# dwu4/fhe-si

Measured on AMD Instinct MI355X. Metric: homomorphic ciphertext-mults/sec (incl. relinearize) at n=2^14, logQ=512, higher is better.
Workload: dtype u32 (every transformed row is a row of 4-byte residues modulo a prime below 2^30: tensor half over primes of 30 bits, key switch over four of 30; coefficients are u64 limbs)

## Files before the change

fhe-si_amd/csrc/capi_ctx.hip:

```cpp
#include "capi_common.h"

int ws_reserve(fhesi_ctx* ctx, int slot, size_t bytes, void** out) {
  if (ctx->ws_bytes[slot] < bytes) {
    if (ctx->ws[slot]) { HIP_TRY(hipStreamSynchronize(ctx->stream)); HIP_TRY(hipFree(ctx->ws[slot])); ctx->ws[slot] = nullptr; ctx->ws_bytes[slot] = 0; }
    size_t want = bytes + (bytes >> 3) + 4096;
    if (hipMalloc(&ctx->ws[slot], want) != hipSuccess) {
      (void)hipGetLastError();
      ctx->ws[slot] = nullptr;
      if (hipMalloc(&ctx->ws[slot], bytes) != hipSuccess) {
        (void)hipGetLastError();
        ctx->ws[slot] = nullptr;
        ctx->ws_oom = true;
        FHESI_FAIL("workspace slot %d: hipMalloc of %zu bytes failed", slot, bytes);
      }
      want = bytes;
    }
    ctx->ws_bytes[slot] = want;
  }
  *out = ctx->ws[slot];
  if (ctx->ws_poison && bytes) HIP_TRY(hipMemsetAsync(ctx->ws[slot], 0xA5, bytes, ctx->stream));
  return 0;
}

int upload_idx(fhesi_ctx* ctx, const std::vector<int>& idx, int** d_out) {
// ... 34 lines not shown
  twt.assign(n, Shoup2{0, 0});
  for (int i = 0; i < 32; ++i) twt[i] = tw[i];
  for (int u = 0; u < 5; ++u)
    for (int x = 0; x < (1 << u); ++x)
      for (int p1 = 0; p1 < 32; ++p1) twt[32 + ((1 << u) - 1 + x) * 32 + p1] = tw[(1 << (5 + u)) + (p1 << u) + x];
  for (int u = 0; u < R; ++u)
    for (int x = 0; x < (1 << u); ++x)
      for (int jl = 0; jl < 1024; ++jl) twt[1024 + (i64)((1 << u) - 1 + x) * 1024 + jl] = tw[(1 << (10 + u)) + ((i64)hm::brv(jl, 10) << u) + x];
}
static void to_q63(std::vector<Shoup2>& t, u64 q) {
  for (auto& e : t) e.wp = hm::shoup63(e.w, q);
}

thread_local bool g_fhesi_internal_ctx = false;

struct OptDesc { const char* name; const char* env; size_t off; bool wide; };
static const OptDesc kOptions[] = {
  {"ks_direct", "FHESI_KS_DIRECT", offsetof(CtxOptions, ks_direct), false},
  {"ks_residues", "FHESI_KS_RESIDUES", offsetof(CtxOptions, ks_residues), false},
  {"ks_aux60", "FHESI_KS_AUX60", offsetof(CtxOptions, ks_aux60), false},
  {"crt_exact", "FHESI_CRT_EXACT", offsetof(CtxOptions, crt_exact), false},
  {"crt_skip_cleanup", "FHESI_CRT_SKIP_CLEANUP", offsetof(CtxOptions, crt_skip_cleanup), false},
  {"lanes", "FHESI_LANES", offsetof(CtxOptions, lanes), false},
  {"stagger", "FHESI_STAGGER", offsetof(CtxOptions, stagger), false},
  {"batch_chunk", "FHESI_BATCH_CHUNK", offsetof(CtxOptions, batch_chunk), true},
  {"wave_operands", "FHESI_WAVE_OPERANDS", offsetof(CtxOptions, wave_operands), true},
  {"stage_chunk_bytes", "FHESI_STAGE_CHUNK_BYTES", offsetof(CtxOptions, stage_chunk_bytes), true},
  {"wave_single", "FHESI_WAVE_SINGLE", offsetof(CtxOptions, wave_single), false},
  {"tensor32", "FHESI_TENSOR32", offsetof(CtxOptions, tensor32), false},
  {"tensor_bits", "FHESI_TENSOR_BITS", offsetof(CtxOptions, tensor_bits), false},
  {"crt32_mfma", "FHESI_CRT32_MFMA", offsetof(CtxOptions, crt32_mfma), false},
  {"dot32_k4", "FHESI_DOT32_K4", offsetof(CtxOptions, dot32_k4), false},
  {"parts_words", "FHESI_PARTS_WORDS", offsetof(CtxOptions, parts_words), false},
  {"hoist_dot", "FHESI_HOIST_DOT", offsetof(CtxOptions, hoist_dot), false},
  {"automorph_rows", "FHESI_AUTOMORPH_ROWS", offsetof(CtxOptions, automorph_rows), false},
  {"ks_long_keys", "FHESI_KS_LONG_KEYS", offsetof(CtxOptions, ks_long_keys), false},
  {"host_chunk", "FHESI_HOST_CHUNK", offsetof(CtxOptions, host_chunk), true},
  {"host_threads", "FHESI_HOST_THREADS", offsetof(CtxOptions, host_threads), false},
};
static void opt_store(CtxOptions* o, const OptDesc& d, long long v) {
  if (d.wide) *(long long*)((char*)o + d.off) = v; else *(int*)((char*)o + d.off) = (int)v;
}
static long long opt_load(const CtxOptions* o, const OptDesc& d) {
  return d.wide ? *(const long long*)((const char*)o + d.off) : (long long)*(const int*)((const char*)o + d.off);
}
extern "C" int fhesi_ctx_set_option(fhesi_ctx* c, const char* name, int64_t value) {
  if (!c || !name) FHESI_FAIL("set_option: null argument");
  for (const OptDesc& d : kOptions)
    if (!strcmp(d.name, name)) { opt_store(&c->opt, d, value); return 0; }
  FHESI_FAIL("set_option: unknown option '%s'", name);
}
extern "C" int fhesi_ctx_get_option(const fhesi_ctx* c, const char* name, int64_t* value) {
  if (!c || !name || !value) FHESI_FAIL("get_option: null argument");
  for (const OptDesc& d : kOptions)
    if (!strcmp(d.name, name)) { *value = opt_load(&c->opt, d); return 0; }
  FHESI_FAIL("get_option: unknown option '%s'", name);
}
extern "C" int fhesi_ctx_copy_options(fhesi_ctx* dst, const fhesi_ctx* src) {
  if (!dst || !src) FHESI_FAIL("copy_options: null argument");
  dst->opt = src->opt;
  return 0;
}

extern "C" int fhesi_ctx_create(fhesi_ctx** out, int64_t m, int32_t nprimes, const uint64_t* q, const uint64_t* root, int32_t device) {
  if (!out) FHESI_FAIL("null output pointer");
  *out = nullptr;
// ... 317 lines not shown
```

fhe-si_amd/csrc/fhesi_internal.h:

```cpp
#pragma once
#include <hip/hip_runtime.h>
#include <cstdint>
#include <cmath>
#include <cstdio>
#include <map>
#include <string>
#include <atomic>
#include <vector>
#include <algorithm>
#include <type_traits>
#include "hostbig.h"
#include "ct_wide.h"

typedef unsigned int u32;

void fhesi_set_error(const char* fmt, ...);
#define FHESI_FAIL(...) do { fhesi_set_error(__VA_ARGS__); return 1; } while (0)
#define HIP_TRY(expr) do { hipError_t e__ = (expr); if (e__ != hipSuccess) { fhesi_set_error("%s failed: %s (%s:%d)", #expr, hipGetErrorString(e__), __FILE__, __LINE__); return 1; } } while (0)
#define FHESI_OP_SET_ 4
#define FHESI_WS_SLOTS 16
#define FHESI_TRY(expr) do { int r__ = (expr); if (r__) return r__; } while (0)

template <int C, int... Rest, class F> static inline void with_limb_class(int n, F&& f) {
  if constexpr (sizeof...(Rest) == 0) f(std::integral_constant<int, C>{});
// ... 45 lines not shown
  std::vector<u64> P, halfP;
};

struct BluesteinTables;
struct fhesi_aux32;

enum { PROF_NTT_FWD = 0, PROF_NTT_INV = 1, PROF_RNS = 2, PROF_TENSOR = 3, PROF_CRT = 4, PROF_DIGITS = 5, PROF_DOT = 6, PROF_EW = 7, PROF_NTT_FWD_DIGITS_MAIN = 8, PROF_NCLASS = 9,
       PROF_PLAIN_SUM = 15  };
enum { PROF_NAME_CRT_EXACT = PROF_NCLASS, PROF_NAME_KS_RECOMBINE, PROF_NAME_RNS_GENERIC, PROF_NAME_MODSWITCH, PROF_NAME_DIGITS, PROF_NNAME };
struct ProfRec { int cls; double units; hipEvent_t e0, e1; };

struct CtxOptions {
  long long host_chunk = 0;
  int host_threads = 0;
  int ks_long_keys = 0;
  int ks_direct = 0;
  int ks_residues = 0;
  int ks_aux60 = 0;
  int crt_exact = 0;
  int crt_skip_cleanup = 0;
  int lanes = 1;
  int stagger = 0;
  long long batch_chunk = 0;
  long long wave_operands = 0;
  long long stage_chunk_bytes = 0;
  int wave_single = 1;
  int automorph_rows = 0;
  int tensor32 = 1;
  int tensor_bits = 30;
  int crt32_mfma = 1;
  int dot32_k4 = 1;
  int hoist_dot = 0;
  int parts_words = 1;
};

struct fhesi_ctx {
  CtxOptions opt;
  int live_handles = 0;
  int device = 0;
  hipStream_t stream = nullptr;
  hipEvent_t ev0 = nullptr, ev1 = nullptr;
  i64 m = 0, phim = 0;
  int L = 0;
  bool pow2 = false;
  int n_big_primes = 0;
  bool has_small_prime = false;
  int logn = 0;
  i64 lin_q = 0;
  bool lin_prime = false;
  i64 lin_s = 0;
  bool phi_two_term = false;
  int lin_lg = 0;
  std::vector<u64> q, root;
  std::vector<int> zms_idx;
  std::vector<i64> phi;
  std::vector<PrimeConst> pc;
  PrimeConst* d_pc = nullptr;
  Shoup2* d_tw_fwd = nullptr;
  Shoup2* d_tw_inv = nullptr;
  Shoup2* d_twt_fwd = nullptr;
  Shoup2* d_twt_inv = nullptr;
  Shoup2* d_twt_fwd_sub = nullptr;
  Shoup2* d_head_tw = nullptr;
  Shoup2* d_tail_fwd = nullptr;
  Shoup2* d_sub_fold = nullptr;
  int* d_zms_idx = nullptr;
// ... 346 lines not shown
```

fhe-si_amd/csrc/kernels_aux32.hip:

```cpp
#include "fhesi_internal.h"

#include "ntt32_core.inc"

__global__ void __launch_bounds__(256) ntt32_head_kernel(u32* __restrict__ rows, i64 count, int nslots, int a0, Aux32Primes pr, Aux32Head hd) {
  const i64 row = blockIdx.y;
  const int a = a0 + (int)(row % nslots);
  const u32 p = pr.p[a];
  u32* g = rows + row * 2 * A32_N;
  for (i64 e = (i64)blockIdx.x * blockDim.x + threadIdx.x; e < A32_N; e += (i64)gridDim.x * blockDim.x) {
    u32 x = g[e];
    const u32 t = mul_lazy32(g[e + A32_N], hd.head[a], p);
    x = x >= 2 * p ? x - 2 * p : x;
    g[e] = x + t;
    g[e + A32_N] = x + 2 * p - t;
  }
}
__global__ void __launch_bounds__(256) ntt32_tail_kernel(u32* __restrict__ rows, i64 count, int nslots, int a0, Aux32Primes pr, Aux32Head hd) {
  const i64 row = blockIdx.y;
  const int a = a0 + (int)(row % nslots);
  const u32 p = pr.p[a];
  u32* g = rows + row * 2 * A32_N;
  for (i64 e = (i64)blockIdx.x * blockDim.x + threadIdx.x; e < A32_N; e += (i64)gridDim.x * blockDim.x) {
    const u32 A = g[e], B = g[e + A32_N];
    u32 s0 = mul_lazy32(A + B, hd.tail_sum[a], p), s1 = mul_lazy32(A + p - B, hd.tail_dif[a], p);
// ... 59 lines not shown
void aux32_free(fhesi_ctx* ctx) {
  if (!ctx->aux32) return;
  ctx->aux32->tab.release();
  delete ctx->aux32;
  ctx->aux32 = nullptr;
}

int launch_ntt32_fwd(fhesi_ctx* ctx, u32* d_rows, i64 count, int nslots, int a0) {
  FHESI_TRY(aux32_init(ctx));
  if (!count) return 0;
  const fhesi_aux32* x = ctx->aux32;
  const int S = x->S;
  if (S >= 2) { if (!launch_ntt32_head_pass(ctx->stream, S, d_rows, count * nslots, nslots, a0, x->tab)) FHESI_FAIL("ntt32: no kernel for rows of 2^%d", A32_LOGN + S); }
  else if (S) ntt32_head_kernel<<<dim3(16, (unsigned)(count * nslots)), 256, 0, ctx->stream>>>(d_rows, count, nslots, a0, x->pr, x->hd);
  if (S) HIP_TRY(hipGetLastError());
  if (count > 0x7fffffff || (nslots << S) > 65535) FHESI_FAIL("ntt32: too many rows per launch");
  const dim3 grid((unsigned)count, (unsigned)(nslots << S));
  if (!a32_with_S<0, 6>(S, [&](auto s) {
    constexpr int SS = decltype(s)::value;
    PROF_KERNEL(ctx, PROF_NTT_FWD, ntt32_fwd_kernel3<false, SS>);
    ntt32_fwd_kernel3<false, SS><<<grid, A32_T, 0, ctx->stream>>>(d_rows, count, nslots, a0, x->pr, x->tab.d_fwd, Dig32Src{}, x->hd);
  })) FHESI_FAIL("ntt32: no kernel for rows of 2^%d", A32_LOGN + S);
  HIP_TRY(hipGetLastError());
  return 0;
}
int launch_ntt32_inv(fhesi_ctx* ctx, u32* d_rows, i64 count, int nslots, int a0, bool mont, bool tail) {
  FHESI_TRY(aux32_init(ctx));
  if (!count) return 0;
  const fhesi_aux32* x = ctx->aux32;
  const int S = x->S;
  ProfScope prof(ctx, PROF_NTT_INV, (double)(count * nslots));
  if (count > 0x7fffffff || (nslots << S) > 65535) FHESI_FAIL("ntt32: too many rows per launch");
  const dim3 grid((unsigned)count, (unsigned)(nslots << S));
  if (mont && S < 3) { PROF_KERNEL(ctx, PROF_NTT_INV, ntt32_inv_kernel3<true>); ntt32_inv_kernel3<true><<<grid, A32_T, 0, ctx->stream>>>(d_rows, count, nslots, a0, x->pr, x->tab.d_inv, S, nullptr); }
  else { PROF_KERNEL(ctx, PROF_NTT_INV, ntt32_inv_kernel3<false>); ntt32_inv_kernel3<false><<<grid, A32_T, 0, ctx->stream>>>(d_rows, count, nslots, a0, x->pr, x->tab.d_inv, S, nullptr); }
  HIP_TRY(hipGetLastError());
  if (S >= 2 && !tail) FHESI_FAIL("ntt32: rows of 2^16 and longer have no consumer that takes their tail stages");
  if (S && tail) {
    if (S >= 2) { if (!launch_ntt32_tail_pass(ctx->stream, S, d_rows, count * nslots, nslots, a0, x->tab, mont ? 1 : 0)) FHESI_FAIL("ntt32: no kernel for rows of 2^%d", A32_LOGN + S); }
    else ntt32_tail_kernel<<<dim3(16, (unsigned)(count * nslots)), 256, 0, ctx->stream>>>(d_rows, count, nslots, a0, x->pr, x->hd);
    HIP_TRY(hipGetLastError());
  }
  return 0;
}
int aux32_tail_consts(fhesi_ctx* ctx, uint32_t (*tw)[2], uint32_t (*twp)[2]) {
  FHESI_TRY(aux32_init(ctx));
  const fhesi_aux32* x = ctx->aux32;
  for (int a = 0; a < 4; ++a) { tw[a][0] = x->hd.tail_sum[a].w; twp[a][0] = x->hd.tail_sum[a].wp; tw[a][1] = x->hd.tail_dif[a].w; twp[a][1] = x->hd.tail_dif[a].wp; }
  return 0;
}
int launch_ntt32_fwd_digits(fhesi_ctx* ctx, const u64* d_parts, int nl, int digit_bits, int nd, i64 npolys, u32* d_out, i64 sub_units, bool wm) {
  FHESI_TRY(aux32_init(ctx));
  if (!npolys) return 0;
  const fhesi_aux32* x = ctx->aux32;
  const int S = x->S;
  ProfScope prof(ctx, PROF_NTT_FWD, (double)(npolys * nd * 4));
  ProfScope main_prof(ctx, PROF_NTT_FWD_DIGITS_MAIN, (double)(npolys * nd * 4));
  const i64 units = npolys * nd;
  if (units > 0x7fffffff) FHESI_FAIL("ntt32: too many digit rows per launch");
  if (digit_bits > 30) FHESI_FAIL("ntt32: digits of %d bits (the first stage of a digit row assumes values below 2p)", digit_bits);
  Dig32Src src{d_parts, nl, digit_bits, nd, (u32)ctx->phim, (u32)sub_units, div32_inv((u32)nd), div32_inv((u32)sub_units)};
  if (S >= 3) {
    if (!ctx->lin_q) FHESI_FAIL("ntt32: digit rows of 2^%d exist for the padded linear-convolution rings only", A32_LOGN + S);
    if (units > 65535) FHESI_FAIL("ntt32: %lld digit rows of 2^%d in one launch (at least 2 MB each: the caller's chunks are smaller)", (long long)units, A32_LOGN + S);
    void* tmp;
    FHESI_TRY(ws_reserve(ctx, 11, (size_t)units * 4 * ((size_t)A32_N << S) * 4, &tmp));
// ... 658 lines not shown
```

fhe-si_amd/csrc/kernels_tensor32.hip:

```cpp
#include "fhesi_internal.h"
#include "lin_fold.h"
#include "ntt32_core.inc"
#include "crt32_bytes.h"
#include <cmath>

struct T32Config {
  u64 lift = 0;
  int nl = 0, logQ = 0, NP = 0, R = 28, WT = 0;
  bool generic = false;
  T32Primes pr;
  u32* d_rns = nullptr;
  Tw32* d_cinv = nullptr;
  u32* d_inv57 = nullptr;
  u32* d_Mw = nullptr;
  u32* d_bytes = nullptr;
  ~T32Config() { hipFree(d_rns); hipFree(d_cinv); hipFree(d_inv57); hipFree(d_Mw); hipFree(d_bytes); }
};
struct fhesi_tensor32 {
  int S = 0;
  int bits = 30;
  hm::Ring32Consts k;
  Ring32Dev tab;
  std::vector<T32Config*> cfgs;
  T32Config* cur = nullptr;
// ... 664 lines not shown
    default: break;
  }
#undef T32_RNS
  FHESI_FAIL("tensor32: %d limbs", c->nl);
}
template <class F>
static inline void t32_with_bits(const fhesi_tensor32* x, F&& f) {
  if (x->bits == 29) f(std::integral_constant<int, 29>{}); else f(std::integral_constant<int, 30>{});
}
static int t32_fwd(fhesi_ctx* ctx, const T32Config* c, u32* d_r, i64 npolys) {
  const fhesi_tensor32* x = ctx->tensor32;
  ProfScope prof(ctx, PROF_NTT_FWD, (double)(npolys * c->NP));
  if (npolys > 0x7fffffff) FHESI_FAIL("tensor32: too many rows per launch");
  const dim3 grid((unsigned)npolys, (unsigned)(c->NP << x->S));
  if (x->S >= 3) {
    if (!launch_ntt32_head_pass(ctx->stream, x->S, d_r, npolys * c->NP, c->NP, 0, x->tab)) FHESI_FAIL("tensor32: no kernel for rows of 2^%d", A32_LOGN + x->S);
    HIP_TRY(hipGetLastError());
  }
  if (!a32_with_S<0, 6>(x->S, [&](auto s) {
    constexpr int SS = decltype(s)::value;
    t32_with_bits(x, [&](auto pb) {
      constexpr int PB = decltype(pb)::value;
      PROF_KERNEL(ctx, PROF_NTT_FWD, (ntt32_fwd_kernel3<false, SS, false, T32Primes, true, false, PB>));
      ntt32_fwd_kernel3<false, SS, false, T32Primes, true, false, PB><<<grid, A32_T, 0, ctx->stream>>>(d_r, npolys, c->NP, 0, c->pr, x->tab.d_fwd, Dig32Src{}, Aux32Head{});
    });
  })) FHESI_FAIL("tensor32: no kernel for rows of 2^%d", A32_LOGN + x->S);
  HIP_TRY(hipGetLastError());
  return 0;
}
template <bool TENSOR>
static int t32_inv(fhesi_ctx* ctx, const T32Config* c, u32* rows, i64 nrows, dim3 grid, const u32* src) {
  const fhesi_tensor32* x = ctx->tensor32;
  ProfScope prof(ctx, PROF_NTT_INV, (double)(nrows * c->NP));
  t32_with_bits(x, [&](auto pb) {
    constexpr int PB = decltype(pb)::value;
    PROF_KERNEL(ctx, PROF_NTT_INV, (ntt32_inv_kernel3<false, TENSOR, T32Primes, PB>));
    ntt32_inv_kernel3<false, TENSOR, T32Primes, PB><<<grid, A32_T, 0, ctx->stream>>>(rows, nrows, c->NP, 0, c->pr, x->tab.d_inv, x->S, src);
  });
  HIP_TRY(hipGetLastError());
  return 0;
}
template <int LQ, int R, int WT, int S>
static int t32_launch_crt(fhesi_ctx* ctx, const T32Config* c, const u32* d_t, i64 npolys, u64* d_parts, bool wm) {
  if (c->NP > (R == 28 ? T32_NP_28 : T32_NP_26)) FHESI_FAIL("tensor32: %d primes exceed the bound the CRT window is derived from", c->NP);
  const i64 n = (i64)A32_N << S;
  const dim3 grid((unsigned)(n / 128), (unsigned)npolys);
  void* d_fl;
  const size_t nwg = (size_t)grid.x * grid.y, fl_bytes = (nwg + 15) & ~(size_t)15;
  if (nwg > 0x7fffffff) FHESI_FAIL("tensor32: too many rows per launch");
  FHESI_TRY(ws_reserve(ctx, 6, fl_bytes + (size_t)(T32_LIST_HDR + T32_LIST_CAP) * 4, &d_fl));
  unsigned char* fl = (unsigned char*)d_fl;
  u32* list = reinterpret_cast<u32*>(fl + fl_bytes);
  t32_list_clear_kernel<<<1, 64, 0, ctx->stream>>>(list);
  bool mfma = false;
  if constexpr (LQ == 512 && S == 0) mfma = c->d_bytes != nullptr && (ctx->opt.crt32_mfma >= 2 || (ctx->opt.crt32_mfma == 1 && nwg >= T32_MFMA_MIN_WG));
  if (mfma) {
    if constexpr (LQ == 512 && S == 0) {
      const u32 nblk = nwg >= 32 * 2048 ? 32u : (nwg >= 2 * 2048 ? (u32)(nwg / 2048) : 1u);
      PROF_KERNEL(ctx, PROF_CRT, (crt32_mfma_kernel<LQ>));
      crt32_mfma_kernel<LQ><<<(unsigned)((nwg + nblk - 1) / nblk), 256, 0, ctx->stream>>>(d_t, c->NP, c->d_inv57, c->d_bytes, reinterpret_cast<u32*>(d_parts), fl, list, (u32)nwg, nblk, wm ? 1 : 0);
    }
  } else {
    PROF_KERNEL(ctx, PROF_CRT, (crt32_scale_kernel<LQ, false, R, WT, S>));
    crt32_scale_kernel<LQ, false, R, WT, S><<<grid, 128, 0, ctx->stream>>>(d_t, n, c->NP, c->pr, c->d_cinv, c->d_inv57, c->d_Mw, d_parts, fl, list, (u32)npolys, wm ? 1 : 0);
  }
  HIP_TRY(hipGetLastError());
// ... 103 lines not shown
```

fhe-si_amd/csrc/ntt32_core.inc:

```
#pragma once
#include <algorithm>
#include <type_traits>

#include "ring32_tables.h"

struct Aux32Primes { u32 p[4]; u32 ninv[4], ninv_p[4]; u64 pinv64[4] , r64[4] , r48[4] ;
                     u32 mont[4] , ninv_m[4], ninv_m_p[4] ;
                     u32 ninv_mw[4][4], ninv_mw_p[4][4] ; };

struct Aux32Head { Tw32 head[4], tail_sum[4], tail_dif[4];
                   Tw32 head1[4][2]; };
static constexpr int T32_MAXP = 76;
struct T32Primes { u32 p[T32_MAXP], ninv[T32_MAXP], ninv_p[T32_MAXP], mu61[T32_MAXP], ninv_w[T32_MAXP], ninv_w_p[T32_MAXP]; u32 closing; };
static constexpr u32 T32_ROWS_PLAIN = 0, T32_ROWS_CRT = 1;
template <class T, class V>
static inline bool a32_upload(T** d, const V& v) {
  const size_t bytes = v.size() * sizeof(v[0]);
  return hipMalloc((void**)d, bytes) == hipSuccess && hipMemcpy(*d, v.data(), bytes, hipMemcpyHostToDevice) == hipSuccess;
}
struct Ring32Dev {
  Tw32* d_fwd = nullptr;
  Tw32* d_inv = nullptr;
  Tw32* d_ht = nullptr;
  u32* d_p = nullptr;
  Tw32* d_hs = nullptr;
  void release() { hipFree(d_fwd); hipFree(d_inv); hipFree(d_ht); hipFree(d_p); hipFree(d_hs); *this = Ring32Dev(); }
  int upload(const hm::Ring32Tables& t) {
    Ring32Dev n;
    const int S = t.k.S;
    if (!(a32_upload(&n.d_fwd, t.fwd) && a32_upload(&n.d_inv, t.inv) && (S < 2 || (a32_upload(&n.d_ht, t.ht) && a32_upload(&n.d_p, t.k.primes))) &&
          (S < 3 || a32_upload(&n.d_hs, t.hs)))) {
      n.release();
      FHESI_FAIL("30-bit rows: uploading the transform tables of %d primes failed", (int)t.k.primes.size());
    }
// ... 238 lines not shown
  for (int a = 0; a < 4; ++a) {
    u32 v[1 << S];
#pragma unroll
    for (int h = 0; h < (1 << S); ++h) v[h] = dig[h];
    a32_head_net<S>(v, hs + (i64)a * 2 * A32_HSN(S), pr.p[a]);
    u32* g = dst + ((c * 4 + a) << (A32_LOGN + S));
#pragma unroll
    for (int h = 0; h < (1 << S); ++h) g[(i64)h * A32_N + e] = v[h];
  }
}
static constexpr int A32_HR = 16;
static constexpr int A32_TBL = 992;
__device__ __forceinline__ u32 a32_tbl_pos(u32 e) {
  return e;
}
__device__ __forceinline__ void a32_stage_tbl(Tw32* __restrict__ tbl, const Tw32* __restrict__ tab, u32 tid) {
  tbl[a32_tbl_pos(tid)] = tab[32 + tid];
  if (tid < 992 - 512) tbl[a32_tbl_pos(512 + tid)] = tab[32 + 512 + tid];
}
__device__ __forceinline__ u32 a32_tbl_idx(int u, u32 kq, int i) {
  return (32 << u) - 32 + (kq << u) + i;
}
typedef unsigned int a32_v4u __attribute__((ext_vector_type(4)));
#define A32_LOAD_TC(tc, tab, v, tid, wv, lane)                                                                              \
  {                                                                                                                         \
    const u32 so_ = ((1024u << (v)) * 8u) + (((wv) << (v)) * 1024u);                                                        \
    _Pragma("unroll") for (int q_ = 0; q_ < (1 << (v)); ++q_) {                                                             \
      const a32_v4u x_ = __builtin_amdgcn_raw_buffer_load_b128(tab, lane, so_ + q_ * 1024u, 0);                             \
      const int i0_ = 2 * q_, i1_ = 2 * q_ + 1;                                                                             \
      tc[i0_ >> (v)][i0_ & ((1 << (v)) - 1)] = Tw32{x_.x, x_.y};                                                  \
      tc[i1_ >> (v)][i1_ & ((1 << (v)) - 1)] = Tw32{x_.z, x_.w};                                                  \
    }                                                                                                                       \
  }
template <bool DIGITS, int S, bool PAD = false, class PR = Aux32Primes, bool NEGW = true, bool WM = false, int PB = 30>
#ifndef A32_FWD_WAVES
#define A32_FWD_WAVES 6
#endif
#ifndef A32_FWD_WAVES_S1
#define A32_FWD_WAVES_S1 6
#endif
__global__ void __launch_bounds__(A32_T, (DIGITS && ((S == 1 && !PAD) || S == 2)) ? A32_FWD_WAVES_S1 : A32_FWD_WAVES) ntt32_fwd_kernel3(
    u32* __restrict__ rows, i64 count, int nslots, int a0, PR pr, const Tw32* __restrict__ tabs,
                                                              Dig32Src ds, Aux32Head hd) {
  static_assert(PB == 30 || (PB == 29 && !DIGITS && NEGW), "primes below 2^29: plain rows of the tensor half");
  __shared__ u32 lds[A32_HR * A32_P];
  __shared__ Tw32 tbl[A32_TBL];
  const u32 tid = threadIdx.x;
  i64 c = blockIdx.x;
  int ps = (int)blockIdx.y;
  if (DIGITS) {
    const u32 bid = blockIdx.x;
    ps = (int)((bid >> 3) & ((4u << S) - 1));
    c = (i64)(bid >> (5 + S)) * 8 + (bid & 7);
    if (c >= count) return;
  }
  const int slot = ps >> S, h = ps & ((1 << S) - 1);
  const int a = a0 + slot;
  const u32 p = pr.p[a];
  const Tw32* __restrict__ tab = tabs + (((i64)a << S) + h) * A32_N;
  u32* __restrict__ g = rows + ((((c * nslots + slot)) << S) + h) * A32_N;
  a32_stage_tbl(tbl, tab, tid);
  u32 r[32];
  if constexpr (DIGITS && S >= 3) {
    const u32* __restrict__ srow = reinterpret_cast<const u32*>(ds.parts) + ((((c * 4 + slot)) << S) + h) * (i64)A32_N;
#pragma unroll
    for (int k = 0; k < 32; ++k) r[k] = srow[k * A32_T + tid];
// ... 147 lines not shown
      u32* w = stage + ((sub & 1) * 8 + (lo >> 1)) * 72 + (lo & 1) * 36;
#pragma unroll
      for (int i = 0; i < 32; ++i) {
        u32 v = r[i];
        if (!DIGITS) {
          const u32 twop = 2 * p;
          if (PB == 29) v = min(v, v - 2 * twop);
          v = v >= twop ? v - twop : v; v = v >= p ? v - p : v;
        }
        w[i] = v;
      }
    }
    __builtin_amdgcn_wave_barrier();
    const u32 pos = lane < 32 ? lane : lane + 4;
    i64 cnt_s = count, c_s = c, base_s = 0;
    if (DIGITS && ds.sub_units) {
      const i64 sub = div32((u32)c, ds.sub_units, ds.sub_inv), rest = count - sub * ds.sub_units;
      c_s = c - sub * ds.sub_units;
      cnt_s = rest < (i64)ds.sub_units ? rest : (i64)ds.sub_units;
      base_s = sub * ds.sub_units * (((i64)4 << (A32_LOGN - 6 + S)) * 64);
    }
    const i64 stride = DIGITS ? cnt_s * 64 : 64;
    u32* __restrict__ sp = (DIGITS ? rows + base_s + ((((i64)a << (A32_LOGN - 6 + S)) + ((i64)h << (A32_LOGN - 6)) + (32 * wv + 16 * hh)) * cnt_s + c_s) * 64 : g + (32 * wv + 16 * hh) * 64);
    const u32 lboff = lane * 4;
#pragma unroll
    for (int t = 0; t < 16; ++t) {
      const u32 v = stage[t * 72 + pos];
      st32(sp, lboff, v);
      sp += stride;
    }
  }
}

template <bool MONT, bool TENSOR = false, class PR = Aux32Primes, int PB = 30>
__global__ void __launch_bounds__(A32_T, A32_INV_WAVES) ntt32_inv_kernel3(u32* __restrict__ rows, i64 count, int nslots, int a0, PR pr, const Tw32* __restrict__ tabs, int S,
                                                              const u32* __restrict__ tsrc) {
  static_assert(PB == 30 || (PB == 29 && !MONT), "primes below 2^29: the rows of the tensor half");
  __shared__ u32 lds[A32_HR * A32_P];
  __shared__ Tw32 tbl[A32_TBL];
  const u32 tid = threadIdx.x;
  i64 c = blockIdx.x;
  const int ps = (int)blockIdx.y;
  if (TENSOR && count >= 24) {
    const u32 bid = blockIdx.x;
    const u32 grp = bid / 24, in = bid % 24;
    const i64 ct = (i64)grp * 8 + (in & 7);
    c = ct * 3 + (in >> 3);
    if (ct * 3 >= count) return;
  }
  const int slot = ps >> S, h = ps & ((1 << S) - 1), a = a0 + slot;
  const u32 p = pr.p[a];
  const Tw32* __restrict__ tab = tabs + (((i64)a << S) + h) * A32_N;
  u32* __restrict__ g = rows + (((c * nslots + slot) << S) + h) * A32_N;
  const u32 kq = tid >> 4, lo = tid & 15, wv = TENSOR ? tid >> 6 : __builtin_amdgcn_readfirstlane(tid >> 6), sub = kq & 3, lane = tid & 63;
  const bool upper = kq >= A32_HR;
  a32_stage_tbl(tbl, tab, tid);
  u32 r[32];
  u32* __restrict__ stage = lds + 2 * wv * A32_P;
#pragma unroll
  for (int hh = 0; hh < 2; ++hh) {
    const u32 pos = lane < 32 ? lane : lane + 4;
    u32 v[16];
    if constexpr (TENSOR) {
      const i64 ct = c / 3;
      const int comp = (int)(c - ct * 3);
      auto srow = [&](int jj) { return tsrc + (((((ct * 4 + jj) * nslots + slot)) << S) + h) * A32_N; };
      const u32* __restrict__ sa = srow(comp == 2 ? 1 : 0);
      const u32* __restrict__ sb = srow(comp == 0 ? 2 : 3);
      const u32 mu = pr.mu61[a], twop = 2 * p;
      auto red = [&](u64 x) -> u32 {
        const u32 q = __umulhi((u32)(x >> (PB == 29 ? 28 : 29)), mu);
        const u32 r = (u32)x - q * p;
        return r >= twop ? r - twop : r;
      };
      if (comp == 1) {
        const u32* __restrict__ sc = srow(1);
        const u32* __restrict__ sd = srow(2);
#pragma unroll
        for (int t0 = 0; t0 < 16; t0 += 8) {
          u32 x0[8], y1[8], x1[8], y0[8];
#pragma unroll
          for (int t = 0; t < 8; ++t) {
            const u32 off = ((4 * wv + 2 * hh + ((t0 + t) >> 3)) * 8 + ((t0 + t) & 7)) * 64 + lane;
            x0[t] = sa[off]; y1[t] = sb[off]; x1[t] = sc[off]; y0[t] = sd[off];
          }
#pragma unroll
          for (int t = 0; t < 8; ++t) v[t0 + t] = red((u64)x0[t] * y1[t] + (u64)x1[t] * y0[t]);
        }
      } else {
        u32 x[16], y[16];
#pragma unroll
        for (int t = 0; t < 16; ++t) {
          const u32 off = ((4 * wv + 2 * hh + (t >> 3)) * 8 + (t & 7)) * 64 + lane;
          x[t] = sa[off]; y[t] = sb[off];
        }
#pragma unroll
        for (int t = 0; t < 16; ++t) v[t] = red((u64)x[t] * y[t]);
      }
    } else {
#pragma unroll
      for (int t = 0; t < 16; ++t) v[t] = g[((4 * wv + 2 * hh + (t >> 3)) * 8 + (t & 7)) * 64 + lane];
    }
    __builtin_amdgcn_wave_barrier();
#pragma unroll
    for (int t = 0; t < 16; ++t) stage[t * 72 + pos] = v[t];
    __builtin_amdgcn_wave_barrier();
    if ((int)(sub >> 1) == hh) {
      const u32* w = stage + ((sub & 1) * 8 + (lo >> 1)) * 72 + (lo & 1) * 36;
#pragma unroll
      for (int i = 0; i < 32; ++i) r[i] = w[i];
    }
  }
  const u32 tcb = lane * 16, wvs = __builtin_amdgcn_readfirstlane(tid >> 6);
  const __amdgpu_buffer_rsrc_t tabr = __builtin_amdgcn_make_buffer_rsrc(const_cast<Tw32*>(tab), 0, A32_N * 8, 0x00020000);
#pragma unroll
  for (int v = 3; v >= 0; --v) {
    const int h = 8 >> v;
    Tw32 tc[2][8];
    A32_LOAD_TC(tc, A32_TABC, v, tid, wvs, tcb);
#pragma unroll
    for (int gq = 0; gq < 2; ++gq) {
#pragma unroll
      for (int b = 0; b < 8; ++b) {
        const int x = a32_bfly_k(b, h);
        if (MONT && !TENSOR && v == 3) a32_gs<true>(r[gq * 16 + x], r[gq * 16 + x + h], tc[gq][x >> (4 - v)], p);
        else if (PB == 29) a32_gs29(r[gq * 16 + x], r[gq * 16 + x + h], tc[gq][x >> (4 - v)], p, v == 3 || (x & (h >> 1)) != 0);
        else a32_gs(r[gq * 16 + x], r[gq * 16 + x + h], tc[gq][x >> (4 - v)], p);
      }
    }
  }
  {
    u32* __restrict__ row = lds + (2 * wv + (sub & 1)) * A32_P;
#pragma unroll
    for (int hh = 0; hh < 2; ++hh) {
      __builtin_amdgcn_wave_barrier();
      if ((int)(sub >> 1) == hh) {
#pragma unroll
        for (int i = 0; i < 32; ++i) row[lo * 36 + i] = r[i];
      }
      __builtin_amdgcn_wave_barrier();
      if ((int)(sub >> 1) == hh) {
#pragma unroll
        for (int k2 = 0; k2 < 32; ++k2) r[k2] = row[a32_f(k2 * 16 + lo)];
      }
    }
  }
  __syncthreads();
#pragma unroll
  for (int u = 4; u >= 0; --u) {
    const int h = 16 >> u;
    Tw32 tb[16];
#pragma unroll
    for (int i = 0; i < (1 << u); ++i) tb[i] = tbl[a32_tbl_idx(u, kq, i)];
#pragma unroll
    for (int b = 0; b < 16; ++b) {
      const int k2 = a32_bfly_k(b, h);
      if (PB == 29) a32_gs29(r[k2], r[k2 + h], tb[k2 >> (5 - u)], p, u != 4 && (k2 & (h >> 1)) != 0);
      else a32_gs(r[k2], r[k2 + h], tb[k2 >> (5 - u)], p);
    }
  }
  u32 t[16];
  if (!upper) {
#pragma unroll
    for (int k2 = 0; k2 < 32; ++k2) lds[kq * A32_P + a32_f(k2 * 16 + lo)] = r[k2];
  }
  __syncthreads();
#pragma unroll
  for (int k = 0; k < 16; ++k) t[k] = lds[k * A32_P + a32_f(tid)];
  __syncthreads();
  if (upper) {
#pragma unroll
    for (int k2 = 0; k2 < 32; ++k2) lds[(kq - A32_HR) * A32_P + a32_f(k2 * 16 + lo)] = r[k2];
  }
  __syncthreads();
#pragma unroll
  for (int k = 0; k < 16; ++k) r[16 + k] = lds[k * A32_P + a32_f(tid)];
#define R(k) ((k) < 16 ? t[(k)] : r[(k)])
#pragma unroll
  for (int s2 = 4; s2 >= 1; --s2) {
    const int h = 16 >> s2;
#pragma unroll
    for (int b = 0; b < 16; ++b) {
      const int k = a32_bfly_k(b, h);
      if (PB == 29) a32_gs29<true>(R(k), R(k + h), tab[(1 << s2) + (k >> (5 - s2))], p, s2 != 4 && (k & (h >> 1)) != 0);
      else a32_gs<false, true>(R(k), R(k + h), tab[(1 << s2) + (k >> (5 - s2))], p);
    }
  }
  Tw32 tn, tnw;
  if constexpr (MONT) { tn = Tw32{pr.ninv_m[a], pr.ninv_m_p[a]}; tnw = Tw32{pr.ninv_mw[a][h], pr.ninv_mw_p[a][h]}; }
  else if constexpr (std::is_same<PR, T32Primes>::value) {
    if (pr.closing) { tn = Tw32{pr.ninv[a], pr.ninv_p[a]}; tnw = Tw32{pr.ninv_w[a], pr.ninv_w_p[a]}; } else { tn = tab[0]; tnw = tab[1]; }
  }
  else { tn = tab[0]; tnw = tab[1]; }
  auto mulc = [&](u32 y, Tw32 t) -> u32 {
    const u32 Q = __umulhi(y, t.wp);
    return (u32)mad64(Q, 0u - p, mul64_s(y, t.w));
  };
#pragma unroll
  for (int k = 0; k < 16; ++k) {
    const u32 sm = t[k] + r[k + 16], df = t[k] - r[k + 16] + ((PB == 29 && !(k & 8)) ? 4 * p : 2 * p);
    u32 v0 = mulc(sm, tn), v1 = mulc(df, tnw);
    v0 = min(v0, v0 - p); v1 = min(v1, v1 - p);
    g[k * A32_T + tid] = v0;
    g[(k + 16) * A32_T + tid] = v1;
  }
#undef R
}
```

Measured before the change: 33050.

## Add persistent row-walking inverse NTT kernel that stages twiddle table once per block

Adds a persistent variant of the 32-bit inverse NTT in which each block is sized to resident occupancy and loops over a contiguous range of rows for one prime. The LDS twiddle table is staged once per block instead of once per row, and launch and tail overhead are amortised. The kernel body moves to a shared include with a WALK template flag, and the path is on by default for S==0 in the aux and tensor-half inverse transforms. In exchange it adds an extra block barrier per row and gives up the tensor path's interleaved block ordering, which may reduce cache locality of the source rows. It also falls back to the old kernel when there are too few rows per prime.

```diff
diff --git a/fhe-si_amd/csrc/capi_ctx.hip b/fhe-si_amd/csrc/capi_ctx.hip
--- a/fhe-si_amd/csrc/capi_ctx.hip
+++ b/fhe-si_amd/csrc/capi_ctx.hip
@@ -90,6 +90,7 @@
   {"crt32_mfma", "FHESI_CRT32_MFMA", offsetof(CtxOptions, crt32_mfma), false},
   {"dot32_k4", "FHESI_DOT32_K4", offsetof(CtxOptions, dot32_k4), false},
   {"parts_words", "FHESI_PARTS_WORDS", offsetof(CtxOptions, parts_words), false},
+  {"rows_walk", "FHESI_ROWS_WALK", offsetof(CtxOptions, rows_walk), false},
   {"hoist_dot", "FHESI_HOIST_DOT", offsetof(CtxOptions, hoist_dot), false},
   {"automorph_rows", "FHESI_AUTOMORPH_ROWS", offsetof(CtxOptions, automorph_rows), false},
   {"ks_long_keys", "FHESI_KS_LONG_KEYS", offsetof(CtxOptions, ks_long_keys), false},
diff --git a/fhe-si_amd/csrc/fhesi_internal.h b/fhe-si_amd/csrc/fhesi_internal.h
--- a/fhe-si_amd/csrc/fhesi_internal.h
+++ b/fhe-si_amd/csrc/fhesi_internal.h
@@ -101,6 +101,7 @@
   int dot32_k4 = 1;
   int hoist_dot = 0;
   int parts_words = 1;
+  int rows_walk = 1;
 };
 
 struct fhesi_ctx {
diff --git a/fhe-si_amd/csrc/kernels_aux32.hip b/fhe-si_amd/csrc/kernels_aux32.hip
--- a/fhe-si_amd/csrc/kernels_aux32.hip
+++ b/fhe-si_amd/csrc/kernels_aux32.hip
@@ -115,6 +115,21 @@
   ProfScope prof(ctx, PROF_NTT_INV, (double)(count * nslots));
   if (count > 0x7fffffff || (nslots << S) > 65535) FHESI_FAIL("ntt32: too many rows per launch");
   const dim3 grid((unsigned)count, (unsigned)(nslots << S));
+  if (S == 0 && ctx->opt.rows_walk) {
+    auto go = [&](auto kernel, int slots) -> int {
+      if (slots < 0) FHESI_FAIL("ntt32: the runtime gives no occupancy for the row-walking inverse kernel");
+      const int W = a32_walk_groups(ctx, slots, count, nslots);
+      if (!W) return -1;
+      prof_kernel(ctx, PROF_NTT_INV, (const void*)kernel);
+      kernel<<<dim3((unsigned)W, (unsigned)nslots), A32_T, 0, ctx->stream>>>(d_rows, count, nslots, a0, x->pr, x->tab.d_inv, nullptr);
+      HIP_TRY(hipGetLastError());
+      return 0;
+    };
+    constexpr auto walk_m = ntt32_inv_walk_kernel3<true>;
+    constexpr auto walk_p = ntt32_inv_walk_kernel3<false>;
+    const int rc = mont ? go(walk_m, a32_resident_slots<walk_m>(ctx->device)) : go(walk_p, a32_resident_slots<walk_p>(ctx->device));
+    if (rc >= 0) return rc;
+  }
   if (mont && S < 3) { PROF_KERNEL(ctx, PROF_NTT_INV, ntt32_inv_kernel3<true>); ntt32_inv_kernel3<true><<<grid, A32_T, 0, ctx->stream>>>(d_rows, count, nslots, a0, x->pr, x->tab.d_inv, S, nullptr); }
   else { PROF_KERNEL(ctx, PROF_NTT_INV, ntt32_inv_kernel3<false>); ntt32_inv_kernel3<false><<<grid, A32_T, 0, ctx->stream>>>(d_rows, count, nslots, a0, x->pr, x->tab.d_inv, S, nullptr); }
   HIP_TRY(hipGetLastError());
diff --git a/fhe-si_amd/csrc/kernels_tensor32.hip b/fhe-si_amd/csrc/kernels_tensor32.hip
--- a/fhe-si_amd/csrc/kernels_tensor32.hip
+++ b/fhe-si_amd/csrc/kernels_tensor32.hip
@@ -720,6 +720,18 @@
 static int t32_inv(fhesi_ctx* ctx, const T32Config* c, u32* rows, i64 nrows, dim3 grid, const u32* src) {
   const fhesi_tensor32* x = ctx->tensor32;
   ProfScope prof(ctx, PROF_NTT_INV, (double)(nrows * c->NP));
+  if (x->S == 0 && x->bits == 30 && ctx->opt.rows_walk) {
+    constexpr auto walk = ntt32_inv_walk_kernel3<false, TENSOR, T32Primes>;
+    const int slots = a32_resident_slots<walk>(ctx->device);
+    if (slots < 0) FHESI_FAIL("tensor32: the runtime gives no occupancy for the row-walking inverse kernel");
+    if (nrows > 0x7fffffff) FHESI_FAIL("tensor32: too many rows per launch");
+    if (const int W = a32_walk_groups(ctx, slots, nrows, c->NP)) {
+      prof_kernel(ctx, PROF_NTT_INV, (const void*)walk);
+      walk<<<dim3((unsigned)W, (unsigned)c->NP), A32_T, 0, ctx->stream>>>(rows, nrows, c->NP, 0, c->pr, x->tab.d_inv, src);
+      HIP_TRY(hipGetLastError());
+      return 0;
+    }
+  }
   t32_with_bits(x, [&](auto pb) {
     constexpr int PB = decltype(pb)::value;
     PROF_KERNEL(ctx, PROF_NTT_INV, (ntt32_inv_kernel3<false, TENSOR, T32Primes, PB>));
diff --git a/fhe-si_amd/csrc/ntt32_core.inc b/fhe-si_amd/csrc/ntt32_core.inc
--- a/fhe-si_amd/csrc/ntt32_core.inc
+++ b/fhe-si_amd/csrc/ntt32_core.inc
@@ -1,5 +1,6 @@
 #pragma once
 #include <algorithm>
+#include <atomic>
 #include <type_traits>
 
 #include "ring32_tables.h"
@@ -304,6 +305,26 @@
       tc[i1_ >> (v)][i1_ & ((1 << (v)) - 1)] = Tw32{x_.z, x_.w};                                                  \
     }                                                                                                                       \
   }
+__device__ __forceinline__ void a32_walk_range(u32 w, u32 W, u32 count, u32& c0, u32& c1) {
+  const u32 base = __builtin_amdgcn_readfirstlane(count / W), rem = count - base * W;
+  c0 = w * base + min(w, rem);
+  c1 = w < W ? c0 + base + (w < rem ? 1u : 0u) : c0;
+}
+template <bool WALK>
+__device__ __forceinline__ u32 a32_row_tid(u32 tid, u32 wave) {
+  if constexpr (WALK) {
+    u32 zero = 0;
+    asm volatile("" : "+s"(wave), "+s"(zero));
+    const u32 lane = __builtin_amdgcn_mbcnt_hi(~0u, __builtin_amdgcn_mbcnt_lo(~0u, zero));
+    return ((wave & (A32_T / 64 - 1)) << 6) | (lane & 63);
+  }
+  return tid;
+}
+template <bool WALK>
+__device__ __forceinline__ i64 a32_row_index(i64 c) {
+  if constexpr (WALK) { u32 cu = (u32)c; asm volatile("" : "+s"(cu)); return (i64)cu; }
+  return c;
+}
 template <bool DIGITS, int S, bool PAD = false, class PR = Aux32Primes, bool NEGW = true, bool WM = false, int PB = 30>
 #ifndef A32_FWD_WAVES
 #define A32_FWD_WAVES 6
@@ -517,177 +538,38 @@
   }
 }
 
+template <auto KERNEL>
+static inline int a32_resident_slots(int device) {
+  static std::atomic<int> slots[64];
+  if (device < 0 || device >= 64) return -1;
+  int s = slots[device].load(std::memory_order_relaxed);
+  if (!s) {
+    int per_cu = 0, cus = 0;
+    if (hipOccupancyMaxActiveBlocksPerMultiprocessor(&per_cu, KERNEL, A32_T, 0) != hipSuccess || per_cu < 1 ||
+        hipDeviceGetAttribute(&cus, hipDeviceAttributeMultiprocessorCount, device) != hipSuccess || cus < 1) return -1;
+    s = per_cu * cus;
+    slots[device].store(s, std::memory_order_relaxed);
+  }
+  return s;
+}
+static constexpr i64 A32_WALK_MIN_ROWS = 4;
+static inline int a32_walk_groups(const fhesi_ctx* ctx, int slots, i64 rows_per_prime, int nslots) {
+  if (ctx->opt.rows_walk == 0) return 0;
+  const int W = std::max(1, slots / nslots);
+  if (ctx->opt.rows_walk != 2 && rows_per_prime < A32_WALK_MIN_ROWS * W) return 0;
+  return W;
+}
+
 template <bool MONT, bool TENSOR = false, class PR = Aux32Primes, int PB = 30>
 __global__ void __launch_bounds__(A32_T, A32_INV_WAVES) ntt32_inv_kernel3(u32* __restrict__ rows, i64 count, int nslots, int a0, PR pr, const Tw32* __restrict__ tabs, int S,
                                                               const u32* __restrict__ tsrc) {
-  static_assert(PB == 30 || (PB == 29 && !MONT), "primes below 2^29: the rows of the tensor half");
-  __shared__ u32 lds[A32_HR * A32_P];
-  __shared__ Tw32 tbl[A32_TBL];
-  const u32 tid = threadIdx.x;
-  i64 c = blockIdx.x;
-  const int ps = (int)blockIdx.y;
-  if (TENSOR && count >= 24) {
-    const u32 bid = blockIdx.x;
-    const u32 grp = bid / 24, in = bid % 24;
-    const i64 ct = (i64)grp * 8 + (in & 7);
-    c = ct * 3 + (in >> 3);
-    if (ct * 3 >= count) return;
-  }
-  const int slot = ps >> S, h = ps & ((1 << S) - 1), a = a0 + slot;
-  const u32 p = pr.p[a];
-  const Tw32* __restrict__ tab = tabs + (((i64)a << S) + h) * A32_N;
-  u32* __restrict__ g = rows + (((c * nslots + slot) << S) + h) * A32_N;
-  const u32 kq = tid >> 4, lo = tid & 15, wv = TENSOR ? tid >> 6 : __builtin_amdgcn_readfirstlane(tid >> 6), sub = kq & 3, lane = tid & 63;
-  const bool upper = kq >= A32_HR;
-  a32_stage_tbl(tbl, tab, tid);
-  u32 r[32];
-  u32* __restrict__ stage = lds + 2 * wv * A32_P;
-#pragma unroll
-  for (int hh = 0; hh < 2; ++hh) {
-    const u32 pos = lane < 32 ? lane : lane + 4;
-    u32 v[16];
-    if constexpr (TENSOR) {
-      const i64 ct = c / 3;
-      const int comp = (int)(c - ct * 3);
-      auto srow = [&](int jj) { return tsrc + (((((ct * 4 + jj) * nslots + slot)) << S) + h) * A32_N; };
-      const u32* __restrict__ sa = srow(comp == 2 ? 1 : 0);
-      const u32* __restrict__ sb = srow(comp == 0 ? 2 : 3);
-      const u32 mu = pr.mu61[a], twop = 2 * p;
-      auto red = [&](u64 x) -> u32 {
-        const u32 q = __umulhi((u32)(x >> (PB == 29 ? 28 : 29)), mu);
-        const u32 r = (u32)x - q * p;
-        return r >= twop ? r - twop : r;
-      };
-      if (comp == 1) {
-        const u32* __restrict__ sc = srow(1);
-        const u32* __restrict__ sd = srow(2);
-#pragma unroll
-        for (int t0 = 0; t0 < 16; t0 += 8) {
-          u32 x0[8], y1[8], x1[8], y0[8];
-#pragma unroll
-          for (int t = 0; t < 8; ++t) {
-            const u32 off = ((4 * wv + 2 * hh + ((t0 + t) >> 3)) * 8 + ((t0 + t) & 7)) * 64 + lane;
-            x0[t] = sa[off]; y1[t] = sb[off]; x1[t] = sc[off]; y0[t] = sd[off];
-          }
-#pragma unroll
-          for (int t = 0; t < 8; ++t) v[t0 + t] = red((u64)x0[t] * y1[t] + (u64)x1[t] * y0[t]);
-        }
-      } else {
-        u32 x[16], y[16];
-#pragma unroll
-        for (int t = 0; t < 16; ++t) {
-          const u32 off = ((4 * wv + 2 * hh + (t >> 3)) * 8 + (t & 7)) * 64 + lane;
-          x[t] = sa[off]; y[t] = sb[off];
-        }
-#pragma unroll
-        for (int t = 0; t < 16; ++t) v[t] = red((u64)x[t] * y[t]);
-      }
-    } else {
-#pragma unroll
-      for (int t = 0; t < 16; ++t) v[t] = g[((4 * wv + 2 * hh + (t >> 3)) * 8 + (t & 7)) * 64 + lane];
-    }
-    __builtin_amdgcn_wave_barrier();
-#pragma unroll
-    for (int t = 0; t < 16; ++t) stage[t * 72 + pos] = v[t];
-    __builtin_amdgcn_wave_barrier();
-    if ((int)(sub >> 1) == hh) {
-      const u32* w = stage + ((sub & 1) * 8 + (lo >> 1)) * 72 + (lo & 1) * 36;
-#pragma unroll
-      for (int i = 0; i < 32; ++i) r[i] = w[i];
-    }
-  }
-  const u32 tcb = lane * 16, wvs = __builtin_amdgcn_readfirstlane(tid >> 6);
-  const __amdgpu_buffer_rsrc_t tabr = __builtin_amdgcn_make_buffer_rsrc(const_cast<Tw32*>(tab), 0, A32_N * 8, 0x00020000);
-#pragma unroll
-  for (int v = 3; v >= 0; --v) {
-    const int h = 8 >> v;
-    Tw32 tc[2][8];
-    A32_LOAD_TC(tc, A32_TABC, v, tid, wvs, tcb);
-#pragma unroll
-    for (int gq = 0; gq < 2; ++gq) {
-#pragma unroll
-      for (int b = 0; b < 8; ++b) {
-        const int x = a32_bfly_k(b, h);
-        if (MONT && !TENSOR && v == 3) a32_gs<true>(r[gq * 16 + x], r[gq * 16 + x + h], tc[gq][x >> (4 - v)], p);
-        else if (PB == 29) a32_gs29(r[gq * 16 + x], r[gq * 16 + x + h], tc[gq][x >> (4 - v)], p, v == 3 || (x & (h >> 1)) != 0);
-        else a32_gs(r[gq * 16 + x], r[gq * 16 + x + h], tc[gq][x >> (4 - v)], p);
-      }
-    }
-  }
-  {
-    u32* __restrict__ row = lds + (2 * wv + (sub & 1)) * A32_P;
-#pragma unroll
-    for (int hh = 0; hh < 2; ++hh) {
-      __builtin_amdgcn_wave_barrier();
-      if ((int)(sub >> 1) == hh) {
-#pragma unroll
-        for (int i = 0; i < 32; ++i) row[lo * 36 + i] = r[i];
-      }
-      __builtin_amdgcn_wave_barrier();
-      if ((int)(sub >> 1) == hh) {
-#pragma unroll
-        for (int k2 = 0; k2 < 32; ++k2) r[k2] = row[a32_f(k2 * 16 + lo)];
-      }
-    }
-  }
-  __syncthreads();
-#pragma unroll
-  for (int u = 4; u >= 0; --u) {
-    const int h = 16 >> u;
-    Tw32 tb[16];
-#pragma unroll
-    for (int i = 0; i < (1 << u); ++i) tb[i] = tbl[a32_tbl_idx(u, kq, i)];
-#pragma unroll
-    for (int b = 0; b < 16; ++b) {
-      const int k2 = a32_bfly_k(b, h);
-      if (PB == 29) a32_gs29(r[k2], r[k2 + h], tb[k2 >> (5 - u)], p, u != 4 && (k2 & (h >> 1)) != 0);
-      else a32_gs(r[k2], r[k2 + h], tb[k2 >> (5 - u)], p);
-    }
-  }
-  u32 t[16];
-  if (!upper) {
-#pragma unroll
-    for (int k2 = 0; k2 < 32; ++k2) lds[kq * A32_P + a32_f(k2 * 16 + lo)] = r[k2];
-  }
-  __syncthreads();
-#pragma unroll
-  for (int k = 0; k < 16; ++k) t[k] = lds[k * A32_P + a32_f(tid)];
-  __syncthreads();
-  if (upper) {
-#pragma unroll
-    for (int k2 = 0; k2 < 32; ++k2) lds[(kq - A32_HR) * A32_P + a32_f(k2 * 16 + lo)] = r[k2];
-  }
-  __syncthreads();
-#pragma unroll
-  for (int k = 0; k < 16; ++k) r[16 + k] = lds[k * A32_P + a32_f(tid)];
-#define R(k) ((k) < 16 ? t[(k)] : r[(k)])
-#pragma unroll
-  for (int s2 = 4; s2 >= 1; --s2) {
-    const int h = 16 >> s2;
-#pragma unroll
-    for (int b = 0; b < 16; ++b) {
-      const int k = a32_bfly_k(b, h);
-      if (PB == 29) a32_gs29<true>(R(k), R(k + h), tab[(1 << s2) + (k >> (5 - s2))], p, s2 != 4 && (k & (h >> 1)) != 0);
-      else a32_gs<false, true>(R(k), R(k + h), tab[(1 << s2) + (k >> (5 - s2))], p);
-    }
-  }
-  Tw32 tn, tnw;
-  if constexpr (MONT) { tn = Tw32{pr.ninv_m[a], pr.ninv_m_p[a]}; tnw = Tw32{pr.ninv_mw[a][h], pr.ninv_mw_p[a][h]}; }
-  else if constexpr (std::is_same<PR, T32Primes>::value) {
-    if (pr.closing) { tn = Tw32{pr.ninv[a], pr.ninv_p[a]}; tnw = Tw32{pr.ninv_w[a], pr.ninv_w_p[a]}; } else { tn = tab[0]; tnw = tab[1]; }
-  }
-  else { tn = tab[0]; tnw = tab[1]; }
-  auto mulc = [&](u32 y, Tw32 t) -> u32 {
-    const u32 Q = __umulhi(y, t.wp);
-    return (u32)mad64(Q, 0u - p, mul64_s(y, t.w));
-  };
-#pragma unroll
-  for (int k = 0; k < 16; ++k) {
-    const u32 sm = t[k] + r[k + 16], df = t[k] - r[k + 16] + ((PB == 29 && !(k & 8)) ? 4 * p : 2 * p);
-    u32 v0 = mulc(sm, tn), v1 = mulc(df, tnw);
-    v0 = min(v0, v0 - p); v1 = min(v1, v1 - p);
-    g[k * A32_T + tid] = v0;
-    g[(k + 16) * A32_T + tid] = v1;
-  }
-#undef R
-}
+  constexpr bool WALK = false;
+#include "ntt32_inv_body.inc"
+}
+template <bool MONT, bool TENSOR = false, class PR = Aux32Primes>
+__global__ void __launch_bounds__(A32_T, A32_INV_WAVES) ntt32_inv_walk_kernel3(u32* __restrict__ rows, i64 count, int nslots, int a0, PR pr, const Tw32* __restrict__ tabs,
+                                                                               const u32* __restrict__ tsrc) {
+  constexpr int S = 0, PB = 30;
+  constexpr bool WALK = true;
+#include "ntt32_inv_body.inc"
+}
diff --git a/fhe-si_amd/csrc/ntt32_inv_body.inc b/fhe-si_amd/csrc/ntt32_inv_body.inc
--- /dev/null
+++ b/fhe-si_amd/csrc/ntt32_inv_body.inc
@@ -0,0 +1,181 @@
+  static_assert(PB == 30 || (PB == 29 && !MONT), "primes below 2^29: the rows of the tensor half");
+  __shared__ u32 lds[A32_HR * A32_P];
+  __shared__ Tw32 tbl[A32_TBL];
+  const u32 tid0 = threadIdx.x, wave0 = __builtin_amdgcn_readfirstlane(tid0 >> 6);
+  i64 c_row = blockIdx.x;
+  const int ps = (int)blockIdx.y;
+  u32 c_end = 0;
+  if constexpr (WALK) {
+    u32 c0;
+    a32_walk_range(blockIdx.x, gridDim.x, (u32)count, c0, c_end);
+    if (c0 >= c_end) return;
+    c_row = c0;
+  } else if (TENSOR && count >= 24) {
+    const u32 bid = blockIdx.x;
+    const u32 grp = bid / 24, in = bid % 24;
+    const i64 ct = (i64)grp * 8 + (in & 7);
+    c_row = ct * 3 + (in >> 3);
+    if (ct * 3 >= count) return;
+  }
+  const int slot = ps >> S, h = ps & ((1 << S) - 1), a = a0 + slot;
+  const u32 p = pr.p[a];
+  const Tw32* __restrict__ tab = tabs + (((i64)a << S) + h) * A32_N;
+  a32_stage_tbl(tbl, tab, tid0);
+  do {
+  const u32 tid = a32_row_tid<WALK>(tid0, wave0);
+  const i64 c = a32_row_index<WALK>(c_row);
+  const u32 kq = tid >> 4, lo = tid & 15, wv = TENSOR ? tid >> 6 : __builtin_amdgcn_readfirstlane(tid >> 6), sub = kq & 3, lane = tid & 63;
+  const bool upper = kq >= A32_HR;
+  u32* __restrict__ g = rows + (((c * nslots + slot) << S) + h) * A32_N;
+  u32 r[32];
+  u32* __restrict__ stage = lds + 2 * wv * A32_P;
+#pragma unroll
+  for (int hh = 0; hh < 2; ++hh) {
+    const u32 pos = lane < 32 ? lane : lane + 4;
+    u32 v[16];
+    if constexpr (TENSOR) {
+      const i64 ct = c / 3;
+      const int comp = (int)(c - ct * 3);
+      auto srow = [&](int jj) { return tsrc + (((((ct * 4 + jj) * nslots + slot)) << S) + h) * A32_N; };
+      const u32* __restrict__ sa = srow(comp == 2 ? 1 : 0);
+      const u32* __restrict__ sb = srow(comp == 0 ? 2 : 3);
+      const u32 mu = pr.mu61[a], twop = 2 * p;
+      auto red = [&](u64 x) -> u32 {
+        const u32 q = __umulhi((u32)(x >> (PB == 29 ? 28 : 29)), mu);
+        const u32 r = (u32)x - q * p;
+        return r >= twop ? r - twop : r;
+      };
+      if (comp == 1) {
+        const u32* __restrict__ sc = srow(1);
+        const u32* __restrict__ sd = srow(2);
+#pragma unroll
+        for (int t0 = 0; t0 < 16; t0 += 8) {
+          u32 x0[8], y1[8], x1[8], y0[8];
+#pragma unroll
+          for (int t = 0; t < 8; ++t) {
+            const u32 off = ((4 * wv + 2 * hh + ((t0 + t) >> 3)) * 8 + ((t0 + t) & 7)) * 64 + lane;
+            x0[t] = sa[off]; y1[t] = sb[off]; x1[t] = sc[off]; y0[t] = sd[off];
+          }
+#pragma unroll
+          for (int t = 0; t < 8; ++t) v[t0 + t] = red((u64)x0[t] * y1[t] + (u64)x1[t] * y0[t]);
+        }
+      } else {
+        u32 x[16], y[16];
+#pragma unroll
+        for (int t = 0; t < 16; ++t) {
+          const u32 off = ((4 * wv + 2 * hh + (t >> 3)) * 8 + (t & 7)) * 64 + lane;
+          x[t] = sa[off]; y[t] = sb[off];
+        }
+#pragma unroll
+        for (int t = 0; t < 16; ++t) v[t] = red((u64)x[t] * y[t]);
+      }
+    } else {
+#pragma unroll
+      for (int t = 0; t < 16; ++t) v[t] = g[((4 * wv + 2 * hh + (t >> 3)) * 8 + (t & 7)) * 64 + lane];
+    }
+    if constexpr (WALK) { if (hh == 0) __syncthreads(); }
+    __builtin_amdgcn_wave_barrier();
+#pragma unroll
+    for (int t = 0; t < 16; ++t) stage[t * 72 + pos] = v[t];
+    __builtin_amdgcn_wave_barrier();
+    if ((int)(sub >> 1) == hh) {
+      const u32* w = stage + ((sub & 1) * 8 + (lo >> 1)) * 72 + (lo & 1) * 36;
+#pragma unroll
+      for (int i = 0; i < 32; ++i) r[i] = w[i];
+    }
+  }
+  const u32 tcb = lane * 16, wvs = __builtin_amdgcn_readfirstlane(tid >> 6);
+  const __amdgpu_buffer_rsrc_t tabr = __builtin_amdgcn_make_buffer_rsrc(const_cast<Tw32*>(tab), 0, A32_N * 8, 0x00020000);
+#pragma unroll
+  for (int v = 3; v >= 0; --v) {
+    const int h = 8 >> v;
+    Tw32 tc[2][8];
+    A32_LOAD_TC(tc, A32_TABC, v, tid, wvs, tcb);
+#pragma unroll
+    for (int gq = 0; gq < 2; ++gq) {
+#pragma unroll
+      for (int b = 0; b < 8; ++b) {
+        const int x = a32_bfly_k(b, h);
+        if (MONT && !TENSOR && v == 3) a32_gs<true>(r[gq * 16 + x], r[gq * 16 + x + h], tc[gq][x >> (4 - v)], p);
+        else if (PB == 29) a32_gs29(r[gq * 16 + x], r[gq * 16 + x + h], tc[gq][x >> (4 - v)], p, v == 3 || (x & (h >> 1)) != 0);
+        else a32_gs(r[gq * 16 + x], r[gq * 16 + x + h], tc[gq][x >> (4 - v)], p);
+      }
+    }
+  }
+  {
+    u32* __restrict__ row = lds + (2 * wv + (sub & 1)) * A32_P;
+#pragma unroll
+    for (int hh = 0; hh < 2; ++hh) {
+      __builtin_amdgcn_wave_barrier();
+      if ((int)(sub >> 1) == hh) {
+#pragma unroll
+        for (int i = 0; i < 32; ++i) row[lo * 36 + i] = r[i];
+      }
+      __builtin_amdgcn_wave_barrier();
+      if ((int)(sub >> 1) == hh) {
+#pragma unroll
+        for (int k2 = 0; k2 < 32; ++k2) r[k2] = row[a32_f(k2 * 16 + lo)];
+      }
+    }
+  }
+  __syncthreads();
+#pragma unroll
+  for (int u = 4; u >= 0; --u) {
+    const int h = 16 >> u;
+    Tw32 tb[16];
+#pragma unroll
+    for (int i = 0; i < (1 << u); ++i) tb[i] = tbl[a32_tbl_idx(u, kq, i)];
+#pragma unroll
+    for (int b = 0; b < 16; ++b) {
+      const int k2 = a32_bfly_k(b, h);
+      if (PB == 29) a32_gs29(r[k2], r[k2 + h], tb[k2 >> (5 - u)], p, u != 4 && (k2 & (h >> 1)) != 0);
+      else a32_gs(r[k2], r[k2 + h], tb[k2 >> (5 - u)], p);
+    }
+  }
+  u32 t[16];
+  if (!upper) {
+#pragma unroll
+    for (int k2 = 0; k2 < 32; ++k2) lds[kq * A32_P + a32_f(k2 * 16 + lo)] = r[k2];
+  }
+  __syncthreads();
+#pragma unroll
+  for (int k = 0; k < 16; ++k) t[k] = lds[k * A32_P + a32_f(tid)];
+  __syncthreads();
+  if (upper) {
+#pragma unroll
+    for (int k2 = 0; k2 < 32; ++k2) lds[(kq - A32_HR) * A32_P + a32_f(k2 * 16 + lo)] = r[k2];
+  }
+  __syncthreads();
+#pragma unroll
+  for (int k = 0; k < 16; ++k) r[16 + k] = lds[k * A32_P + a32_f(tid)];
+#define R(k) ((k) < 16 ? t[(k)] : r[(k)])
+#pragma unroll
+  for (int s2 = 4; s2 >= 1; --s2) {
+    const int h = 16 >> s2;
+#pragma unroll
+    for (int b = 0; b < 16; ++b) {
+      const int k = a32_bfly_k(b, h);
+      if (PB == 29) a32_gs29<true>(R(k), R(k + h), tab[(1 << s2) + (k >> (5 - s2))], p, s2 != 4 && (k & (h >> 1)) != 0);
+      else a32_gs<false, true>(R(k), R(k + h), tab[(1 << s2) + (k >> (5 - s2))], p);
+    }
+  }
+  Tw32 tn, tnw;
+  if constexpr (MONT) { tn = Tw32{pr.ninv_m[a], pr.ninv_m_p[a]}; tnw = Tw32{pr.ninv_mw[a][h], pr.ninv_mw_p[a][h]}; }
+  else if constexpr (std::is_same<PR, T32Primes>::value) {
+    if (pr.closing) { tn = Tw32{pr.ninv[a], pr.ninv_p[a]}; tnw = Tw32{pr.ninv_w[a], pr.ninv_w_p[a]}; } else { tn = tab[0]; tnw = tab[1]; }
+  }
+  else { tn = tab[0]; tnw = tab[1]; }
+  auto mulc = [&](u32 y, Tw32 t) -> u32 {
+    const u32 Q = __umulhi(y, t.wp);
+    return (u32)mad64(Q, 0u - p, mul64_s(y, t.w));
+  };
+#pragma unroll
+  for (int k = 0; k < 16; ++k) {
+    const u32 sm = t[k] + r[k + 16], df = t[k] - r[k + 16] + ((PB == 29 && !(k & 8)) ? 4 * p : 2 * p);
+    u32 v0 = mulc(sm, tn), v1 = mulc(df, tnw);
+    v0 = min(v0, v0 - p); v1 = min(v1, v1 - p);
+    g[k * A32_T + tid] = v0;
+    g[(k + 16) * A32_T + tid] = v1;
+  }
+  } while (WALK && ++c_row < (i64)c_end);
+#undef R
```

Result: slower. 31810 (-3.7%).
